# josebeo2016/SCL-Deepfake-audio-detection

Hardware: AMD Instinct MI355X
Metric: train-step utterances/sec (64000-sample clips) (higher is better)
Workload: dtype bf16

## Files before the change

### scl-deepfake-audio-detection_amd/csrc/norm.hip

```cpp
#include "common.h"

namespace {

constexpr int MAXCH = 4;

template <bool F32>
__device__ __forceinline__ void load8(const void* base, int64_t off, float (&v)[8]) {
    if (F32) {
        const float4 a = *reinterpret_cast<const float4*>(reinterpret_cast<const float*>(base) + off);
        const float4 b = *reinterpret_cast<const float4*>(reinterpret_cast<const float*>(base) + off + 4);
        v[0] = a.x; v[1] = a.y; v[2] = a.z; v[3] = a.w; v[4] = b.x; v[5] = b.y; v[6] = b.z; v[7] = b.w;
    } else {
        const uint4 u = *reinterpret_cast<const uint4*>(reinterpret_cast<const bf16_t*>(base) + off);
        const uint32_t w[4] = {u.x, u.y, u.z, u.w};
#pragma unroll
        for (int i = 0; i < 4; ++i) {
            v[2 * i] = __uint_as_float(w[i] << 16);
            v[2 * i + 1] = __uint_as_float(w[i] & 0xFFFF0000u);
        }
    }
}
__device__ __forceinline__ void store8_bf16(bf16_t* base, int64_t off, const float (&v)[8]) {
    uint4 u;
    u.x = pack_bf2(v[0], v[1]); u.y = pack_bf2(v[2], v[3]); u.z = pack_bf2(v[4], v[5]); u.w = pack_bf2(v[6], v[7]);
    *reinterpret_cast<uint4*>(base + off) = u;
}
__device__ __forceinline__ void store8_f32(float* base, int64_t off, const float (&v)[8]) {
    *reinterpret_cast<float4*>(base + off) = make_float4(v[0], v[1], v[2], v[3]);
    *reinterpret_cast<float4*>(base + off + 4) = make_float4(v[4], v[5], v[6], v[7]);
}

template <bool XF32, int NR>
__global__ __launch_bounds__(256) void ln_fwd_kernel(const void* __restrict__ x, const float* __restrict__ gamma,
                                                     const float* __restrict__ beta, bf16_t* __restrict__ y_bf,
                                                     float* __restrict__ y_f32, float* __restrict__ mean_out,
                                                     float* __restrict__ rstd_out, int M, int C, int64_t ldx,
                                                     int64_t ldy, float eps, int act) {
    const int lane = threadIdx.x & 63;
    const int row0 = (blockIdx.x * 4 + (threadIdx.x >> 6)) * NR;
    if (row0 >= M) return;
    constexpr int NCHR = NR == 1 ? MAXCH : 2;
    float v[NR][NCHR][8];
    float s[NR];
#pragma unroll
    for (int r = 0; r < NR; ++r) {
        s[r] = 0.f;
#pragma unroll
        for (int ch = 0; ch < NCHR; ++ch) {
            const int c = ch * 512 + lane * 8;
#pragma unroll
            for (int i = 0; i < 8; ++i) v[r][ch][i] = 0.f;
            if (c < C && row0 + r < M) load8<XF32>(x, (int64_t)(row0 + r) * ldx + c, v[r][ch]);
        }
    }
    float mean[NR], rstd[NR];
#pragma unroll
    for (int r = 0; r < NR; ++r) {
#pragma unroll
        for (int ch = 0; ch < NCHR; ++ch) {
            const int c = ch * 512 + lane * 8;
            if (c < C) {
#pragma unroll
                for (int i = 0; i < 8; ++i) s[r] += v[r][ch][i];
            }
        }
        mean[r] = wave_sum(s[r]) / (float)C;
        float q = 0.f;
#pragma unroll
        for (int ch = 0; ch < NCHR; ++ch) {
            const int c = ch * 512 + lane * 8;
            if (c < C) {
#pragma unroll
                for (int i = 0; i < 8; ++i) { const float d = v[r][ch][i] - mean[r]; q += d * d; }
            }
        }
        rstd[r] = rsqrtf(wave_sum(q) / (float)C + eps);
    }
#pragma unroll
    for (int ch = 0; ch < NCHR; ++ch) {
        const int c = ch * 512 + lane * 8;
        if (c < C) {
            float g[8], b[8];
            load8<true>(gamma, c, g);
            load8<true>(beta, c, b);
#pragma unroll
            for (int r = 0; r < NR; ++r) {
                const int row = row0 + r;
                if (row < M) {
                    float o[8];
#pragma unroll
                    for (int i = 0; i < 8; ++i) o[i] = (v[r][ch][i] - mean[r]) * rstd[r] * g[i] + b[i];
                    if ((act & 0xFF) == 1) {
#pragma unroll
                        for (int i = 0; i < 8; i += 2) gelu2(o[i], o[i + 1]);
                    }
                    if (y_bf && (act & 0x100)) {
                        float lo[8];
                        uint4 h;
                        h.x = pack_bf2(o[0], o[1]); h.y = pack_bf2(o[2], o[3]); h.z = pack_bf2(o[4], o[5]); h.w = pack_bf2(o[6], o[7]);
                        const unsigned hw[4] = {h.x, h.y, h.z, h.w};
#pragma unroll
                        for (int i = 0; i < 4; ++i) {
                            lo[2 * i] = o[2 * i] - __uint_as_float(hw[i] << 16);
                            lo[2 * i + 1] = o[2 * i + 1] - __uint_as_float(hw[i] & 0xFFFF0000u);
                        }
                        bf16_t* dst = y_bf + (int64_t)row * 3 * C + c;
                        *reinterpret_cast<uint4*>(dst) = h;
                        *reinterpret_cast<uint4*>(dst + C) = h;
                        store8_bf16(dst, 2 * (int64_t)C, lo);
                    } else if (y_bf) store8_bf16(y_bf, (int64_t)row * ldy + c, o);
                    if (y_f32) store8_f32(y_f32, (int64_t)row * ldy + c, o);
                }
            }
        }
    }
#pragma unroll
    for (int r = 0; r < NR; ++r) {
        if (lane == 0 && row0 + r < M) {
            if (mean_out) mean_out[row0 + r] = mean[r];
            if (rstd_out) rstd_out[row0 + r] = rstd[r];
        }
    }
}

template <bool XF32, bool DYF32, int NCH>
__global__ __launch_bounds__(256, (NCH <= 2 ? 3 : 2)) void ln_bwd_kernel(const void* __restrict__ dy, const void* __restrict__ x,
                                                     const float* __restrict__ mean_in, const float* __restrict__ rstd_in,
                                                     const float* __restrict__ gamma, const float* __restrict__ beta,
                                                     const float* __restrict__ dres, float* __restrict__ dx_f32,
                                                     bf16_t* __restrict__ dx_bf, float* __restrict__ part, int M, int C, int64_t ldx,
                                                     int64_t lddy, int64_t lddx, int rows_per_block, int act, int sum_dres,
                                                     int out_rpb, int64_t out_rbstride, int64_t out_off,
                                                     uint32_t din_seed, float din_p, uint32_t dout_seed, float dout_p) {
    extern __shared__ float red[];
    const int lane = threadIdx.x & 63, w = threadIdx.x >> 6;
    const int r0 = blockIdx.x * rows_per_block;
    const int r1 = min(M, r0 + rows_per_block);
    float ag[NCH][8], ab[NCH][8], ar[NCH][8];
#pragma unroll
    for (int ch = 0; ch < NCH; ++ch)
#pragma unroll
        for (int i = 0; i < 8; ++i) { ag[ch][i] = 0.f; ab[ch][i] = 0.f; ar[ch][i] = 0.f; }
    const int np = 2 + (sum_dres ? 1 : 0);

    for (int row = r0 + w; row < r1; row += 4) {
        const float mean = mean_in[row], rstd = rstd_in[row];
        float xh[NCH][8], dyv[NCH][8];
        float s1 = 0.f, s2 = 0.f;
#pragma unroll
        for (int ch = 0; ch < NCH; ++ch) {
            const int c = ch * 512 + lane * 8;
            if (c < C) {
                float xv[8], g[8];
                load8<XF32>(x, (int64_t)row * ldx + c, xv);
                load8<DYF32>(dy, (int64_t)row * lddy + c, dyv[ch]);
                load8<true>(gamma, c, g);
                if (act == 1) {
                    float b[8];
                    load8<true>(beta, c, b);
                    float gg[8];
#pragma unroll
                    for (int i = 0; i < 8; ++i) gg[i] = ((xv[i] - mean) * rstd) * g[i] + b[i];
#pragma unroll
                    for (int i = 0; i < 8; i += 2) gelu_grad2(gg[i], gg[i + 1]);
#pragma unroll
                    for (int i = 0; i < 8; ++i) dyv[ch][i] *= gg[i];
                }
#pragma unroll
                for (int i = 0; i < 8; ++i) {
                    const float h = (xv[i] - mean) * rstd;
                    xh[ch][i] = h;
                    ag[ch][i] += dyv[ch][i] * h;
                    ab[ch][i] += dyv[ch][i];
                    const float dh = dyv[ch][i] * g[i];
                    dyv[ch][i] = dh;
                    s1 += dh;
                    s2 += dh * h;
                }
            }
        }
        s1 = wave_sum(s1) / (float)C;
        s2 = wave_sum(s2) / (float)C;
#pragma unroll
        for (int ch = 0; ch < NCH; ++ch) {
            const int c = ch * 512 + lane * 8;
            if (c < C) {
                float o[8];
#pragma unroll
                for (int i = 0; i < 8; ++i) o[i] = rstd * (dyv[ch][i] - s1 - xh[ch][i] * s2);
                if (dres) {
                    float r[8];
                    load8<true>(dres, (int64_t)row * lddx + c, r);
#pragma unroll
                    for (int i = 0; i < 8; ++i) {
                        o[i] += r[i];
                        ar[ch][i] += din_p > 0.f ? r[i] * dropout_scale(din_seed, (uint64_t)((int64_t)row * C + c + i), din_p) : r[i];
                    }
                }
                if (sum_dres == 2) {
#pragma unroll
                    for (int i = 0; i < 8; ++i) ar[ch][i] += o[i];
                }
                if (dx_f32) store8_f32(dx_f32, (int64_t)row * lddx + c, o);
                if (dx_bf) {
                    const int64_t orow = out_rpb > 0 ? (int64_t)(row / out_rpb) * out_rbstride + (int64_t)(row % out_rpb) * lddx + out_off
                                                     : (int64_t)row * lddx;
                    if (dout_p > 0.f) {
#pragma unroll
                        for (int i = 0; i < 8; ++i) o[i] *= dropout_scale(dout_seed, (uint64_t)((int64_t)row * C + c + i), dout_p);
                    }
                    store8_bf16(dx_bf, orow + c, o);
                }
            }
        }
    }
#pragma unroll
    for (int ch = 0; ch < NCH; ++ch) {
        const int c = ch * 512 + lane * 8;
        if (c < C) {
#pragma unroll
            for (int i = 0; i < 8; ++i) {
                red[(w * np + 0) * C + c + i] = ag[ch][i];
                red[(w * np + 1) * C + c + i] = ab[ch][i];
                if (sum_dres) red[(w * np + 2) * C + c + i] = ar[ch][i];
            }
        }
    }
    __syncthreads();
    for (int c = threadIdx.x; c < C; c += 256) {
        float g = 0.f, b = 0.f, r = 0.f;
#pragma unroll
        for (int ww = 0; ww < 4; ++ww) {
            g += red[(ww * np + 0) * C + c]; b += red[(ww * np + 1) * C + c];
            if (sum_dres) r += red[(ww * np + 2) * C + c];
        }
        part[(int64_t)blockIdx.x * np * C + c] = g;
        part[(int64_t)blockIdx.x * np * C + C + c] = b;
        if (sum_dres) part[(int64_t)blockIdx.x * np * C + 2 * C + c] = r;
    }
}

__global__ __launch_bounds__(256) void colreduce_kernel(const float* __restrict__ part, float* __restrict__ out, int nparts, int C,
                                                        int64_t pstride, int accumulate) {
    __shared__ float red[8][33];
    const int tx = threadIdx.x & 31, ty = threadIdx.x >> 5;
    const int c = blockIdx.x * 32 + tx;
    float s = 0.f;
    if (c < C)
        for (int p = ty; p < nparts; p += 8) s += part[(int64_t)p * pstride + c];
    red[ty][tx] = s;
    __syncthreads();
    if (ty == 0 && c < C) {
        float t = 0.f;
#pragma unroll
        for (int k = 0; k < 8; ++k) t += red[k][tx];
        out[c] = accumulate ? out[c] + t : t;
    }
}

__global__ __launch_bounds__(256) void colreduce_seg_kernel(const float* __restrict__ part, float* __restrict__ out, int nparts, int C,
                                                            int64_t pstride, int accumulate, float* __restrict__ scratch,
                                                            int* __restrict__ counters, float* __restrict__ out2, int split) {
    __shared__ float red[8][33];
    __shared__ int last_flag;
    const int tx = threadIdx.x & 31, ty = threadIdx.x >> 5;
    const int c = blockIdx.x * 32 + tx;
    const int nseg = gridDim.y, seg = blockIdx.y;
    const int per = (nparts + nseg - 1) / nseg;
    const int p0 = seg * per, p1 = min(nparts, p0 + per);
    float s = 0.f;
    if (c < C)
        for (int p = p0 + ty; p < p1; p += 8) s += part[(int64_t)p * pstride + c];
    red[ty][tx] = s;
    __syncthreads();
    if (ty == 0 && c < C) {
        float t = 0.f;
#pragma unroll
        for (int k = 0; k < 8; ++k) t += red[k][tx];
        __hip_atomic_store(&scratch[(int64_t)seg * C + c], t, __ATOMIC_RELAXED, __HIP_MEMORY_SCOPE_AGENT);
    }
    asm volatile("s_waitcnt vmcnt(0)" ::: "memory");
    __syncthreads();
    if (threadIdx.x == 0) {
        const int t = __hip_atomic_fetch_add(&counters[blockIdx.x], 1, __ATOMIC_RELAXED, __HIP_MEMORY_SCOPE_AGENT);
        const int is_last = t == nseg - 1;
        if (is_last) __hip_atomic_store(&counters[blockIdx.x], 0, __ATOMIC_RELAXED, __HIP_MEMORY_SCOPE_AGENT);
        last_flag = is_last;
    }
    __syncthreads();
    if (last_flag && ty == 0 && c < C) {
        __builtin_amdgcn_fence(__ATOMIC_ACQUIRE, "wavefront");
        float t = 0.f;
        for (int k = 0; k < nseg; ++k) t += __hip_atomic_load(&scratch[(int64_t)k * C + c], __ATOMIC_RELAXED, __HIP_MEMORY_SCOPE_AGENT);
        float* o = (out2 && c >= split) ? out2 + (c - split) : out + c;
        *o = accumulate ? *o + t : t;
    }
}

struct SlabJobs { SclSlabJob job[SCL_SLAB_MAX_JOBS]; int first_block[SCL_SLAB_MAX_JOBS + 1]; int njobs; };
__global__ __launch_bounds__(256) void reduce_slabs_multi_kernel(const SlabJobs J) {
    int j = 0;
    while (j + 1 < J.njobs && (int)blockIdx.x >= J.first_block[j + 1]) ++j;
    const SclSlabJob jb = J.job[j];
    const int nb = J.first_block[j + 1] - J.first_block[j];
    const int64_t i0 = ((int64_t)((int)blockIdx.x - J.first_block[j]) * blockDim.x + threadIdx.x) * 4;
    const int64_t step = (int64_t)nb * blockDim.x * 4;
    for (int64_t i = i0; i < jb.n; i += step) {
        if (i + 4 <= jb.n) {
            float4 s = *reinterpret_cast<const float4*>(jb.slabs + i);
            for (int k = 1; k < jb.nslabs; ++k) {
                const float4 t = *reinterpret_cast<const float4*>(jb.slabs + k * jb.stride + i);
                s.x += t.x; s.y += t.y; s.z += t.z; s.w += t.w;
            }
            *reinterpret_cast<float4*>(jb.out + i) = s;
        } else {
            for (int64_t q = i; q < jb.n; ++q) {
                float s = jb.slabs[q];
                for (int k = 1; k < jb.nslabs; ++k) s += jb.slabs[k * jb.stride + q];
                jb.out[q] = s;
            }
        }
    }
}

struct ReduceJobs { SclReduceJob job[SCL_REDUCE_MAX_JOBS]; int first_block[SCL_REDUCE_MAX_JOBS + 1]; int njobs; };
__global__ __launch_bounds__(1024) void colreduce_multi_kernel(const ReduceJobs J) {
    __shared__ float red[32][33];
    int j = 0;
    while (j + 1 < J.njobs && (int)blockIdx.x >= J.first_block[j + 1]) ++j;
    const SclReduceJob jb = J.job[j];
    const int tx = threadIdx.x & 31, ty = threadIdx.x >> 5;
    const int c = ((int)blockIdx.x - J.first_block[j]) * 32 + tx;
    float s = 0.f;
    if (c < jb.C) {
        int p = ty;
        for (; p + 96 < jb.nparts; p += 128) {
            const float a0 = jb.part[(int64_t)p * jb.pstride + c], a1 = jb.part[(int64_t)(p + 32) * jb.pstride + c];
            const float a2 = jb.part[(int64_t)(p + 64) * jb.pstride + c], a3 = jb.part[(int64_t)(p + 96) * jb.pstride + c];
            s += a0; s += a1; s += a2; s += a3;
        }
        for (; p < jb.nparts; p += 32) s += jb.part[(int64_t)p * jb.pstride + c];
    }
    red[ty][tx] = s;
    __syncthreads();
    if (ty == 0 && c < jb.C) {
        float t = 0.f;
#pragma unroll
        for (int k = 0; k < 32; ++k) t += red[k][tx];
        float* o = (jb.out2 && c >= jb.split) ? jb.out2 + (c - jb.split) : jb.out + c;
        *o = t;
    }
}

template <bool F32>
__global__ __launch_bounds__(256) void colsum_kernel(const void* __restrict__ x, float* __restrict__ part, int M, int N,
                                                     int64_t ld, int rows_per_block, int* __restrict__ counters, float* __restrict__ out) {
    __shared__ float red[16][128 + 1];
    __shared__ int last_flag;
    const int cg = threadIdx.x & 15, ty = threadIdx.x >> 4;
    const int c0 = blockIdx.x * 128 + cg * 8;
    const int r0 = blockIdx.y * rows_per_block, r1 = min(M, r0 + rows_per_block);
    float acc[8] = {0, 0, 0, 0, 0, 0, 0, 0};
    if (c0 < N) {
        for (int r = r0 + ty; r < r1; r += 16) {
            float v[8];
            load8<F32>(x, (int64_t)r * ld + c0, v);
#pragma unroll
            for (int i = 0; i < 8; ++i) acc[i] += v[i];
        }
    }
#pragma unroll
    for (int i = 0; i < 8; ++i) red[ty][cg * 8 + i] = acc[i];
    __syncthreads();
    const int c = blockIdx.x * 128 + threadIdx.x;
    if (threadIdx.x < 128 && c < N) {
        float s = 0.f;
#pragma unroll
        for (int t = 0; t < 16; ++t) s += red[t][threadIdx.x];
        if (out) __hip_atomic_store(&part[(int64_t)blockIdx.y * N + c], s, __ATOMIC_RELAXED, __HIP_MEMORY_SCOPE_AGENT);
        else part[(int64_t)blockIdx.y * N + c] = s;
    }
    if (out == nullptr) return;
    asm volatile("s_waitcnt vmcnt(0)" ::: "memory");
    __syncthreads();
    if (threadIdx.x == 0) {
        const int t = __hip_atomic_fetch_add(&counters[blockIdx.x], 1, __ATOMIC_RELAXED, __HIP_MEMORY_SCOPE_AGENT);
        const int is_last = t == (int)gridDim.y - 1;
        if (is_last) __hip_atomic_store(&counters[blockIdx.x], 0, __ATOMIC_RELAXED, __HIP_MEMORY_SCOPE_AGENT);
        last_flag = is_last;
    }
    __syncthreads();
    if (last_flag) {
        __builtin_amdgcn_fence(__ATOMIC_ACQUIRE, "wavefront");
        const int cc = threadIdx.x & 127, half = threadIdx.x >> 7, ny = gridDim.y;
        const int col = blockIdx.x * 128 + cc;
        float s = 0.f;
        if (col < N) {
            for (int p0 = half; p0 < ny; p0 += 16) {
                float v[8];
#pragma unroll
                for (int j = 0; j < 8; ++j) {
                    const int p = p0 + 2 * j;
                    v[j] = p < ny ? __hip_atomic_load(&part[(int64_t)p * N + col], __ATOMIC_RELAXED, __HIP_MEMORY_SCOPE_AGENT) : 0.f;
                }
#pragma unroll
                for (int j = 0; j < 8; ++j) s += v[j];
            }
        }
        float* flat = &red[0][0];
        flat[threadIdx.x] = s;
        __syncthreads();
        if (threadIdx.x < 128 && col < N) out[col] = flat[threadIdx.x] + flat[threadIdx.x + 128];
    }
}

}

extern "C" int scl_layernorm_fwd(const void* x, int x_f32, const float* gamma, const float* beta, void* y_bf16,
                                 float* y_f32, float* mean, float* rstd, int M, int C, int64_t ldx, int64_t ldy,
                                 float eps, int act, void* stream) {
    SCL_REQUIRE(x && gamma && beta && (y_bf16 || y_f32), "layernorm_fwd: null pointer");
    SCL_REQUIRE(M > 0 && C >= 8 && C <= 2048 && (C & 7) == 0 && (ldx & 7) == 0 && (ldy & 7) == 0,
                "layernorm_fwd: need 8 <= C <= 2048, C, ldx, ldy multiples of 8 (C=%d)", C);
    dim3 block(256);
    hipStream_t s = (hipStream_t)stream;
    const int nr_env = 2;
    const int nr = (nr_env == 2 && C <= 1024 && M >= 4096) ? 2 : 1;
    dim3 grid((M + 4 * nr - 1) / (4 * nr));
#define LN_FWD(XF, NR) hipLaunchKernelGGL((ln_fwd_kernel<XF, NR>), grid, block, 0, s, x, gamma, beta, (bf16_t*)y_bf16, y_f32, mean, rstd, M, C, ldx, ldy, eps, act)
    if (x_f32) { if (nr == 2) LN_FWD(true, 2); else LN_FWD(true, 1); }
    else { if (nr == 2) LN_FWD(false, 2); else LN_FWD(false, 1); }
#undef LN_FWD
    return scl_check_launch("scl_layernorm_fwd");
}

static int ln_bwd_rows_per_block(int M) {
    int rpb = (M + 767) / 768;
    rpb = (rpb + 3) / 4 * 4;
    if (rpb < 4) rpb = 4;
    while ((M + rpb - 1) / rpb > 1024) rpb *= 2;
    return rpb;
}
extern "C" int scl_layernorm_bwd_nparts(int M) {
    const int rpb = ln_bwd_rows_per_block(M);
    return (M + rpb - 1) / rpb;
}

extern "C" int scl_layernorm_bwd(const void* dy, int dy_f32, const void* x, int x_f32, const float* mean,
                                 const float* rstd, const float* gamma, const float* beta, const float* dres,
                                 float* dx_f32, void* dx_bf16, float* part, int M, int C,
                                 int64_t ldx, int64_t lddy, int64_t lddx, int act, int sum_dres, int out_rpb, int64_t out_rbstride,
                                 int64_t out_off, uint32_t din_seed, float din_p, uint32_t dout_seed, float dout_p, void* stream) {
    SCL_REQUIRE(din_p >= 0.f && din_p < 1.f && dout_p >= 0.f && dout_p < 1.f, "layernorm_bwd: dropout probabilities in [0, 1)");
    SCL_REQUIRE(din_p == 0.f || sum_dres == 1, "layernorm_bwd: din mask applies to the column sums of dres (sum_dres = 1)");
    SCL_REQUIRE(dout_p == 0.f || (dx_bf16 && out_rpb == 0 && lddx == C), "layernorm_bwd: dout mask needs a plain [M, C] bf16 output");
    SCL_REQUIRE(out_rpb == 0 || (dx_bf16 && out_rpb > 0 && (out_rbstride & 7) == 0 && (out_off & 7) == 0), "layernorm_bwd: padded output needs dx_bf16");
    SCL_REQUIRE(sum_dres == 0 || (sum_dres == 1 && dres) || (sum_dres == 2 && !dres), "layernorm_bwd: sum_dres 1 needs dres, 2 excludes it");
    SCL_REQUIRE(dy && x && mean && rstd && gamma && part && (dx_f32 || dx_bf16), "layernorm_bwd: null pointer");
    SCL_REQUIRE(act == 0 || beta, "layernorm_bwd: gelu variant needs beta");
    SCL_REQUIRE(M > 0 && C >= 8 && C <= 2048 && (C & 7) == 0 && (ldx & 7) == 0 && (lddy & 7) == 0 && (lddx & 7) == 0,
                "layernorm_bwd: need 8 <= C <= 2048 and multiples of 8");
    const int rows_per_block = ln_bwd_rows_per_block(M);
    const int nblk = (M + rows_per_block - 1) / rows_per_block;
    const size_t lds = (size_t)4 * (2 + (sum_dres ? 1 : 0)) * C * sizeof(float);
    hipStream_t s = (hipStream_t)stream;
    dim3 grid(nblk), block(256);
#define LN_BWD(XF, DF, NC) hipLaunchKernelGGL((ln_bwd_kernel<XF, DF, NC>), grid, block, lds, s, dy, x, mean, rstd, gamma, beta, dres, \
                                              dx_f32, (bf16_t*)dx_bf16, part, M, C, ldx, lddy, lddx, rows_per_block, act, sum_dres, \
                                              out_rpb, out_rbstride, out_off, din_seed, din_p, dout_seed, dout_p)
#define LN_BWD_C(XF, DF) do { if (C <= 512) LN_BWD(XF, DF, 1); else if (C <= 1024) LN_BWD(XF, DF, 2); else LN_BWD(XF, DF, 4); } while (0)
    if (x_f32 && dy_f32) LN_BWD_C(true, true);
    else if (x_f32) LN_BWD_C(true, false);
    else if (dy_f32) LN_BWD_C(false, true);
    else LN_BWD_C(false, false);
#undef LN_BWD_C
#undef LN_BWD
    return scl_check_launch("scl_layernorm_bwd");
}

extern "C" int scl_colreduce_f32(const float* part, float* out, int nparts, int C, int64_t pstride, int accumulate, void* stream) {
    SCL_REQUIRE(part && out && nparts >= 1 && C >= 1, "colreduce: bad args");
    hipLaunchKernelGGL(colreduce_kernel, dim3((C + 31) / 32), dim3(256), 0, (hipStream_t)stream, part, out, nparts, C, pstride, accumulate);
    return scl_check_launch("scl_colreduce_f32");
}

extern "C" int scl_colreduce_seg_f32(const float* part, float* out, int nparts, int C, int64_t pstride, int accumulate, float* scratch,
                                     int* counters, float* out2, int split, void* stream) {
    SCL_REQUIRE(part && out && scratch && counters && nparts >= 1 && C >= 1, "colreduce_seg: bad args");
    SCL_REQUIRE(!out2 || (split > 0 && split < C), "colreduce_seg: split must lie inside (0, C) when out2 is given");
    SCL_REQUIRE((C + 31) / 32 <= SCL_COLSUM_MAX_GROUPS, "colreduce_seg: C too large for the counter array (%d)", C);
    const int nseg = nparts >= 64 ? SCL_COLREDUCE_SEGMENTS : 1;
    hipLaunchKernelGGL(colreduce_seg_kernel, dim3((C + 31) / 32, nseg), dim3(256), 0, (hipStream_t)stream, part, out, nparts, C, pstride,
                       accumulate, scratch, counters, out2, split);
    return scl_check_launch("scl_colreduce_seg_f32");
}

extern "C" int scl_reduce_slabs_multi(const SclSlabJob* jobs, int njobs, void* stream) {
    SCL_REQUIRE(jobs && njobs >= 1 && njobs <= SCL_SLAB_MAX_JOBS, "reduce_slabs_multi: 1 .. %d jobs", SCL_SLAB_MAX_JOBS);
    SlabJobs J;
    int blocks = 0;
    for (int i = 0; i < njobs; ++i) {
        const SclSlabJob& b = jobs[i];
        SCL_REQUIRE(b.slabs && b.out && b.n > 0 && b.nslabs >= 1, "reduce_slabs_multi: job %d: bad arguments", i);
        SCL_REQUIRE(((uintptr_t)b.slabs & 15) == 0 && ((uintptr_t)b.out & 15) == 0 && (b.stride & 3) == 0, "reduce_slabs_multi: job %d: alignment", i);
        J.job[i] = b;
        J.first_block[i] = blocks;
        int nb = (int)((b.n / 4 + 255) / 256); if (nb > 2048) nb = 2048; if (nb < 1) nb = 1;
        blocks += nb;
    }
    J.first_block[njobs] = blocks;
    J.njobs = njobs;
    hipLaunchKernelGGL(reduce_slabs_multi_kernel, dim3(blocks), dim3(256), 0, (hipStream_t)stream, J);
    return scl_check_launch("scl_reduce_slabs_multi");
}

extern "C" int scl_colreduce_multi(const SclReduceJob* jobs, int njobs, void* stream) {
    SCL_REQUIRE(jobs && njobs >= 1 && njobs <= SCL_REDUCE_MAX_JOBS, "colreduce_multi: 1 .. %d jobs", SCL_REDUCE_MAX_JOBS);
    ReduceJobs J;
    int blocks = 0;
    for (int i = 0; i < njobs; ++i) {
        const SclReduceJob& b = jobs[i];
        SCL_REQUIRE(b.part && b.out && b.nparts >= 1 && b.C >= 1 && b.pstride >= b.C, "colreduce_multi: job %d: bad arguments", i);
        SCL_REQUIRE(!b.out2 || (b.split > 0 && b.split < b.C), "colreduce_multi: job %d: split must lie inside (0, C) when out2 is given", i);
        J.job[i] = b;
        J.first_block[i] = blocks;
        blocks += (b.C + 31) / 32;
    }
    J.first_block[njobs] = blocks;
    J.njobs = njobs;
    hipLaunchKernelGGL(colreduce_multi_kernel, dim3(blocks), dim3(1024), 0, (hipStream_t)stream, J);
    return scl_check_launch("scl_colreduce_multi");
}

static int colsum_rows(int M) {
    int rows_per_block = 256;
    while ((M + rows_per_block - 1) / rows_per_block > 64) rows_per_block *= 2;
    return rows_per_block;
}

static int colsum_reduce_rows(int M, int N) {
    if (N > 128) return colsum_rows(M);
    int rows_per_block = 256;
    while ((M + rows_per_block - 1) / rows_per_block > 512) rows_per_block *= 2;
    return rows_per_block;
}

extern "C" int scl_colsum_reduce_nparts(int M, int N) {
    const int rows_per_block = colsum_reduce_rows(M, N);
    return (M + rows_per_block - 1) / rows_per_block;
}

extern "C" int scl_colsum_nparts(int M) {
    const int rows_per_block = colsum_rows(M);
    return (M + rows_per_block - 1) / rows_per_block;
}

extern "C" int scl_colsum(const void* x, int x_f32, float* part, int M, int N, int64_t ld, void* stream) {
    SCL_REQUIRE(x && part && M > 0 && N > 0 && (N & 7) == 0 && (ld & 7) == 0, "colsum: bad args (N, ld multiples of 8)");
    const int rows_per_block = colsum_rows(M);
    dim3 grid((N + 127) / 128, (M + rows_per_block - 1) / rows_per_block), block(256);
    hipStream_t s = (hipStream_t)stream;
    if (x_f32) hipLaunchKernelGGL((colsum_kernel<true>), grid, block, 0, s, x, part, M, N, ld, rows_per_block, (int*)nullptr, (float*)nullptr);
    else hipLaunchKernelGGL((colsum_kernel<false>), grid, block, 0, s, x, part, M, N, ld, rows_per_block, (int*)nullptr, (float*)nullptr);
    return scl_check_launch("scl_colsum");
}

extern "C" int scl_colsum_reduce(const void* x, int x_f32, float* part, int* counters, float* out, int M, int N, int64_t ld, void* stream) {
    SCL_REQUIRE(x && part && counters && out && M > 0 && N > 0 && (N & 7) == 0 && (ld & 7) == 0, "colsum_reduce: bad args (N, ld multiples of 8)");
    SCL_REQUIRE((N + 127) / 128 <= SCL_COLSUM_MAX_GROUPS, "colsum_reduce: N too large for the counter array (%d)", N);
    const int rows_per_block = colsum_reduce_rows(M, N);
    dim3 grid((N + 127) / 128, (M + rows_per_block - 1) / rows_per_block), block(256);
    hipStream_t s = (hipStream_t)stream;
    if (x_f32) hipLaunchKernelGGL((colsum_kernel<true>), grid, block, 0, s, x, part, M, N, ld, rows_per_block, counters, out);
    else hipLaunchKernelGGL((colsum_kernel<false>), grid, block, 0, s, x, part, M, N, ld, rows_per_block, counters, out);
    return scl_check_launch("scl_colsum_reduce");
}
```

Measured before the change: 1626.

## Prefetch next row via buffer loads and move LayerNorm-backward accumulators to LDS

Restructures the LayerNorm backward kernel. Each wave now prefetches the next row's x, dy, dres, mean and rstd with raw buffer loads while it processes the current row. The per-column gamma/beta partial sums move from registers into LDS, and gamma (plus beta for C<=512) is staged in LDS. Template specialisations for C=512/1024 with known output configurations drop the runtime branches. This aims to hide global-load latency and cut register pressure so occupancy can rise, at the cost of extra LDS traffic per row, more LDS per block, and a 2 GiB slab limit from the 32-bit buffer offsets.

Result: no change. 1632, median of 6 (+0.4%).

```diff
diff --git a/scl-deepfake-audio-detection_amd/csrc/norm.hip b/scl-deepfake-audio-detection_amd/csrc/norm.hip
--- a/scl-deepfake-audio-detection_amd/csrc/norm.hip
+++ b/scl-deepfake-audio-detection_amd/csrc/norm.hip
@@ -123,8 +123,47 @@
     }
 }
 
+typedef __attribute__((ext_vector_type(4))) unsigned ln_u32x4;
+__device__ __forceinline__ __amdgpu_buffer_rsrc_t ln_rsrc(const void* base) {
+    return __builtin_amdgcn_make_buffer_rsrc(const_cast<void*>(base), 0, 0xFFFFFFFF, 0x00020000);
+}
+template <bool F32> struct Raw8;
+template <> struct Raw8<true> { ln_u32x4 a, b; };
+template <> struct Raw8<false> { ln_u32x4 u; };
+template <bool F32>
+__device__ __forceinline__ void load8_raw(__amdgpu_buffer_rsrc_t rs, unsigned row_bytes, unsigned c, Raw8<F32>& r) {
+    if constexpr (F32) {
+        r.a = __builtin_amdgcn_raw_buffer_load_b128(rs, c * 4, row_bytes, 0);
+        r.b = __builtin_amdgcn_raw_buffer_load_b128(rs, c * 4 + 16, row_bytes, 0);
+    } else {
+        r.u = __builtin_amdgcn_raw_buffer_load_b128(rs, c * 2, row_bytes, 0);
+    }
+}
+template <bool F32>
+__device__ __forceinline__ void unpack8(const Raw8<F32>& r, float (&v)[8]) {
+    if constexpr (F32) {
+#pragma unroll
+        for (int i = 0; i < 4; ++i) { v[i] = __uint_as_float(r.a[i]); v[4 + i] = __uint_as_float(r.b[i]); }
+    } else {
+        const uint32_t w[4] = {r.u[0], r.u[1], r.u[2], r.u[3]};
+#pragma unroll
+        for (int i = 0; i < 4; ++i) {
+            v[2 * i] = __uint_as_float(w[i] << 16);
+            v[2 * i + 1] = __uint_as_float(w[i] & 0xFFFF0000u);
+        }
+    }
+}
+__device__ __forceinline__ void lds_load8(const float* p, float (&v)[8]) {
+    const float4 a = *reinterpret_cast<const float4*>(p), b = *reinterpret_cast<const float4*>(p + 4);
+    v[0] = a.x; v[1] = a.y; v[2] = a.z; v[3] = a.w; v[4] = b.x; v[5] = b.y; v[6] = b.z; v[7] = b.w;
+}
+constexpr unsigned LN_BWD_AG_UNFUSED = 0x88u;
+
 template <bool XF32, bool DYF32, int NCH>
-__global__ __launch_bounds__(256, (NCH <= 2 ? 3 : 2)) void ln_bwd_kernel(const void* __restrict__ dy, const void* __restrict__ x,
+struct LnBwdRow { Raw8<XF32> x[NCH]; Raw8<DYF32> dy[NCH]; Raw8<true> dres[NCH]; float mean, rstd; };
+
+template <bool XF32, bool DYF32, int NCH, int MODE>
+__global__ __launch_bounds__(256, (NCH == 1 ? 4 : NCH == 2 ? 3 : 2)) void ln_bwd_kernel(const void* __restrict__ dy, const void* __restrict__ x,
                                                      const float* __restrict__ mean_in, const float* __restrict__ rstd_in,
                                                      const float* __restrict__ gamma, const float* __restrict__ beta,
                                                      const float* __restrict__ dres, float* __restrict__ dx_f32,
@@ -132,35 +171,72 @@
                                                      int64_t lddy, int64_t lddx, int rows_per_block, int act, int sum_dres,
                                                      int out_rpb, int64_t out_rbstride, int64_t out_off,
                                                      uint32_t din_seed, float din_p, uint32_t dout_seed, float dout_p) {
-    extern __shared__ float red[];
-    const int lane = threadIdx.x & 63, w = threadIdx.x >> 6;
+    extern __shared__ __attribute__((aligned(16))) float red[];
+    constexpr bool AHEAD = MODE != 0;
+    constexpr bool BETA_LDS = NCH == 1;
+    const bool has_dres = MODE == 1 ? true : MODE == 2 ? false : dres != nullptr;
+    const bool has_f32 = MODE == 1 ? true : MODE == 2 ? false : dx_f32 != nullptr;
+    const bool has_bf = MODE != 0 ? true : dx_bf != nullptr;
+    const bool gelu = MODE == 1 ? false : act == 1;
+    auto in_row = [&](int c) { return MODE != 0 || c < C; };
+    const int lane = threadIdx.x & 63, wv = threadIdx.x >> 6, w = __builtin_amdgcn_readfirstlane(wv);
     const int r0 = blockIdx.x * rows_per_block;
     const int r1 = min(M, r0 + rows_per_block);
-    float ag[NCH][8], ab[NCH][8], ar[NCH][8];
-#pragma unroll
-    for (int ch = 0; ch < NCH; ++ch)
-#pragma unroll
-        for (int i = 0; i < 8; ++i) { ag[ch][i] = 0.f; ab[ch][i] = 0.f; ar[ch][i] = 0.f; }
     const int np = 2 + (sum_dres ? 1 : 0);
-
-    for (int row = r0 + w; row < r1; row += 4) {
-        const float mean = mean_in[row], rstd = rstd_in[row];
+    float* const acc = red + (size_t)w * np * C;
+    float* const gs = red + (size_t)4 * np * C;
+    float* const bs = gs + C;
+    float gb[2][NCH * 2];
+#pragma unroll
+    for (int j = 0; j < NCH * 2; ++j) {
+        const int c = threadIdx.x + 256 * j;
+        if (in_row(c)) {
+            gb[0][j] = gamma[c];
+            if (BETA_LDS && gelu) gb[1][j] = beta[c];
+        }
+    }
+    using Row = LnBwdRow<XF32, DYF32, NCH>;
+    constexpr unsigned XE = XF32 ? 4 : 2, DYE = DYF32 ? 4 : 2;
+    const __amdgpu_buffer_rsrc_t xs = ln_rsrc(reinterpret_cast<const char*>(x) + (int64_t)r0 * ldx * XE);
+    const __amdgpu_buffer_rsrc_t dys = ln_rsrc(reinterpret_cast<const char*>(dy) + (int64_t)r0 * lddy * DYE);
+    const __amdgpu_buffer_rsrc_t drs = ln_rsrc(has_dres ? dres + (int64_t)r0 * lddx : mean_in);
+    const __amdgpu_buffer_rsrc_t ms = ln_rsrc(mean_in + r0), rss = ln_rsrc(rstd_in + r0);
+    const unsigned xrow = (unsigned)ldx * XE, dyrow = (unsigned)lddy * DYE, drrow = (unsigned)lddx * 4;
+    auto load_row = [&](Row& R, int row) {
+        const unsigned rr = (unsigned)(row - r0);
+        R.mean = __uint_as_float(__builtin_amdgcn_raw_buffer_load_b32(ms, 0, rr * 4, 0));
+        R.rstd = __uint_as_float(__builtin_amdgcn_raw_buffer_load_b32(rss, 0, rr * 4, 0));
+#pragma unroll
+        for (int ch = 0; ch < NCH; ++ch) {
+            const int c = ch * 512 + lane * 8;
+            const unsigned cl = in_row(c) ? c : 0;
+            load8_raw<XF32>(xs, rr * xrow, cl, R.x[ch]);
+            load8_raw<DYF32>(dys, rr * dyrow, cl, R.dy[ch]);
+            if (has_dres) load8_raw<true>(drs, rr * drrow, cl, R.dres[ch]);
+        }
+    };
+    auto process = [&](const Row& cur, int row) {
+#pragma clang fp contract(off)
+        const float mean = cur.mean, rstd = cur.rstd;
         float xh[NCH][8], dyv[NCH][8];
         float s1 = 0.f, s2 = 0.f;
 #pragma unroll
         for (int ch = 0; ch < NCH; ++ch) {
             const int c = ch * 512 + lane * 8;
-            if (c < C) {
-                float xv[8], g[8];
-                load8<XF32>(x, (int64_t)row * ldx + c, xv);
-                load8<DYF32>(dy, (int64_t)row * lddy + c, dyv[ch]);
-                load8<true>(gamma, c, g);
-                if (act == 1) {
+            if (in_row(c)) {
+                float xv[8], ag[8], ab[8], g[8];
+                unpack8<XF32>(cur.x[ch], xv);
+                unpack8<DYF32>(cur.dy[ch], dyv[ch]);
+                lds_load8(acc + c, ag);
+                lds_load8(acc + C + c, ab);
+                lds_load8(gs + c, g);
+                if (gelu) {
                     float b[8];
-                    load8<true>(beta, c, b);
+                    if (BETA_LDS) lds_load8(bs + c, b);
+                    else load8<true>(beta, c, b);
                     float gg[8];
 #pragma unroll
-                    for (int i = 0; i < 8; ++i) gg[i] = ((xv[i] - mean) * rstd) * g[i] + b[i];
+                    for (int i = 0; i < 8; ++i) gg[i] = __builtin_fmaf((xv[i] - mean) * rstd, g[i], b[i]);
 #pragma unroll
                     for (int i = 0; i < 8; i += 2) gelu_grad2(gg[i], gg[i + 1]);
 #pragma unroll
@@ -170,13 +246,15 @@
                 for (int i = 0; i < 8; ++i) {
                     const float h = (xv[i] - mean) * rstd;
                     xh[ch][i] = h;
-                    ag[ch][i] += dyv[ch][i] * h;
-                    ab[ch][i] += dyv[ch][i];
+                    ag[i] = ((LN_BWD_AG_UNFUSED >> i) & 1u) ? ag[i] + dyv[ch][i] * h : __builtin_fmaf(dyv[ch][i], h, ag[i]);
+                    ab[i] += dyv[ch][i];
                     const float dh = dyv[ch][i] * g[i];
                     dyv[ch][i] = dh;
                     s1 += dh;
                     s2 += dh * h;
                 }
+                store8_f32(acc, c, ag);
+                store8_f32(acc, C + c, ab);
             }
         }
         s1 = wave_sum(s1) / (float)C;
@@ -184,46 +262,80 @@
 #pragma unroll
         for (int ch = 0; ch < NCH; ++ch) {
             const int c = ch * 512 + lane * 8;
-            if (c < C) {
-                float o[8];
-#pragma unroll
-                for (int i = 0; i < 8; ++i) o[i] = rstd * (dyv[ch][i] - s1 - xh[ch][i] * s2);
-                if (dres) {
+            if (in_row(c)) {
+                float o[8], ar[8];
+                uint64_t e0 = (uint64_t)((int64_t)row * C + c);
+                asm("" : "+v"(e0));
+                if (sum_dres) lds_load8(acc + 2 * C + c, ar);
+#pragma unroll
+                for (int i = 0; i < 8; ++i) o[i] = rstd * __builtin_fmaf(-xh[ch][i], s2, dyv[ch][i] - s1);
+                if (has_dres) {
                     float r[8];
-                    load8<true>(dres, (int64_t)row * lddx + c, r);
+                    unpack8<true>(cur.dres[ch], r);
 #pragma unroll
                     for (int i = 0; i < 8; ++i) {
                         o[i] += r[i];
-                        ar[ch][i] += din_p > 0.f ? r[i] * dropout_scale(din_seed, (uint64_t)((int64_t)row * C + c + i), din_p) : r[i];
+                        ar[i] += din_p > 0.f ? r[i] * dropout_scale(din_seed, e0 + i, din_p) : r[i];
                     }
                 }
                 if (sum_dres == 2) {
 #pragma unroll
-                    for (int i = 0; i < 8; ++i) ar[ch][i] += o[i];
+                    for (int i = 0; i < 8; ++i) ar[i] += o[i];
                 }
-                if (dx_f32) store8_f32(dx_f32, (int64_t)row * lddx + c, o);
-                if (dx_bf) {
+                if (sum_dres) store8_f32(acc, 2 * C + c, ar);
+                if (has_f32) store8_f32(dx_f32, (int64_t)row * lddx + c, o);
+                if (has_bf) {
                     const int64_t orow = out_rpb > 0 ? (int64_t)(row / out_rpb) * out_rbstride + (int64_t)(row % out_rpb) * lddx + out_off
                                                      : (int64_t)row * lddx;
                     if (dout_p > 0.f) {
 #pragma unroll
-                        for (int i = 0; i < 8; ++i) o[i] *= dropout_scale(dout_seed, (uint64_t)((int64_t)row * C + c + i), dout_p);
+                        for (int i = 0; i < 8; ++i) o[i] *= dropout_scale(dout_seed, e0 + i, dout_p);
                     }
                     store8_bf16(dx_bf, orow + c, o);
                 }
             }
         }
+    };
+
+    int row = r0 + w;
+    Row cur, nxt;
+    if (AHEAD && row < r1) load_row(cur, row);
+#pragma unroll
+    for (int j = 0; j < NCH * 2; ++j) {
+        const int c = threadIdx.x + 256 * j;
+        if (in_row(c)) {
+            gs[c] = gb[0][j];
+            if (BETA_LDS && gelu) bs[c] = gb[1][j];
+        }
     }
 #pragma unroll
     for (int ch = 0; ch < NCH; ++ch) {
         const int c = ch * 512 + lane * 8;
-        if (c < C) {
-#pragma unroll
-            for (int i = 0; i < 8; ++i) {
-                red[(w * np + 0) * C + c + i] = ag[ch][i];
-                red[(w * np + 1) * C + c + i] = ab[ch][i];
-                if (sum_dres) red[(w * np + 2) * C + c + i] = ar[ch][i];
-            }
+        if (in_row(c)) {
+            for (int k = 0; k < np; ++k) {
+                *reinterpret_cast<float4*>(acc + k * C + c) = make_float4(0.f, 0.f, 0.f, 0.f);
+                *reinterpret_cast<float4*>(acc + k * C + c + 4) = make_float4(0.f, 0.f, 0.f, 0.f);
+            }
+        }
+    }
+    __syncthreads();
+    if (!AHEAD) {
+        for (; row < r1; row += 4) { load_row(cur, row); process(cur, row); }
+    } else if (row < r1) {
+        if (row + 4 < r1) {
+            load_row(nxt, row + 4);
+            process(cur, row);
+            cur = nxt;
+            row += 4;
+            while (row + 4 < r1) {
+                load_row(nxt, row + 4);
+                process(cur, row);
+                cur = nxt;
+                row += 4;
+            }
+            process(cur, row);
+        } else {
+            process(cur, row);
         }
     }
     __syncthreads();
@@ -461,19 +573,38 @@
     SCL_REQUIRE(M > 0 && C >= 8 && C <= 2048 && (C & 7) == 0 && (ldx & 7) == 0 && (lddy & 7) == 0 && (lddx & 7) == 0,
                 "layernorm_bwd: need 8 <= C <= 2048 and multiples of 8");
     const int rows_per_block = ln_bwd_rows_per_block(M);
+    {
+        const int64_t ldmax = ldx > lddy ? (ldx > lddx ? ldx : lddx) : (lddy > lddx ? lddy : lddx);
+        SCL_REQUIRE((int64_t)rows_per_block * ldmax * 4 < ((int64_t)1 << 31), "layernorm_bwd: a block's slab of rows must stay below 2 GiB");
+    }
     const int nblk = (M + rows_per_block - 1) / rows_per_block;
-    const size_t lds = (size_t)4 * (2 + (sum_dres ? 1 : 0)) * C * sizeof(float);
+    const size_t lds = ((size_t)4 * (2 + (sum_dres ? 1 : 0)) + 1 + (C <= 512 ? 1 : 0)) * C * sizeof(float);
     hipStream_t s = (hipStream_t)stream;
     dim3 grid(nblk), block(256);
-#define LN_BWD(XF, DF, NC) hipLaunchKernelGGL((ln_bwd_kernel<XF, DF, NC>), grid, block, lds, s, dy, x, mean, rstd, gamma, beta, dres, \
+    if (lds > 64 * 1024) {
+        static bool attr_set = false;
+        if (!attr_set) {
+            const int cap = 13 * 2048 * (int)sizeof(float);
+            hipFuncSetAttribute((const void*)ln_bwd_kernel<true, true, 4, 0>, hipFuncAttributeMaxDynamicSharedMemorySize, cap);
+            hipFuncSetAttribute((const void*)ln_bwd_kernel<true, false, 4, 0>, hipFuncAttributeMaxDynamicSharedMemorySize, cap);
+            hipFuncSetAttribute((const void*)ln_bwd_kernel<false, true, 4, 0>, hipFuncAttributeMaxDynamicSharedMemorySize, cap);
+            hipFuncSetAttribute((const void*)ln_bwd_kernel<false, false, 4, 0>, hipFuncAttributeMaxDynamicSharedMemorySize, cap);
+            attr_set = true;
+        }
+    }
+    const bool whole = C == 512 || C == 1024;
+    const int mode = !whole ? 0 : (dres && dx_f32 && dx_bf16 && act != 1) ? 1 : (!dres && !dx_f32 && dx_bf16) ? 2 : 0;
+#define LN_BWD(XF, DF, NC, MD) hipLaunchKernelGGL((ln_bwd_kernel<XF, DF, NC, MD>), grid, block, lds, s, dy, x, mean, rstd, gamma, beta, dres, \
                                               dx_f32, (bf16_t*)dx_bf16, part, M, C, ldx, lddy, lddx, rows_per_block, act, sum_dres, \
                                               out_rpb, out_rbstride, out_off, din_seed, din_p, dout_seed, dout_p)
-#define LN_BWD_C(XF, DF) do { if (C <= 512) LN_BWD(XF, DF, 1); else if (C <= 1024) LN_BWD(XF, DF, 2); else LN_BWD(XF, DF, 4); } while (0)
+#define LN_BWD_M(XF, DF, NC) do { if (mode == 1) LN_BWD(XF, DF, NC, 1); else if (mode == 2) LN_BWD(XF, DF, NC, 2); else LN_BWD(XF, DF, NC, 0); } while (0)
+#define LN_BWD_C(XF, DF) do { if (C <= 512) LN_BWD_M(XF, DF, 1); else if (C <= 1024) LN_BWD_M(XF, DF, 2); else LN_BWD(XF, DF, 4, 0); } while (0)
     if (x_f32 && dy_f32) LN_BWD_C(true, true);
     else if (x_f32) LN_BWD_C(true, false);
     else if (dy_f32) LN_BWD_C(false, true);
     else LN_BWD_C(false, false);
 #undef LN_BWD_C
+#undef LN_BWD_M
 #undef LN_BWD
     return scl_check_launch("scl_layernorm_bwd");
 }
```
